# Cappucciyes/ViT-With-OpenCL

Hardware: AMD Instinct MI355X
Metric: images/sec ViT-B/16 224x224 bs512 (higher is better)
Workload: dtype f32

## Files before the change

### vit-with-opencl_amd/csrc/attention_p3.hip

```cpp
#include "kernelHandler.h"
#include "kernel_limits.h"
#include "vit_kernels.h"
#include "fp32_split.h"
#include "gemm_common.h"

namespace {

constexpr int HD = 64;
constexpr int MAX_LDS = KL_LDS_BYTES;
constexpr int MAX_ROWS = KL_ATTN_HD64_MAX_TOKENS;
static_assert(2 * 2 * 3 * MAX_ROWS * 64 <= MAX_LDS && MAX_ROWS % 16 == 0 && MAX_ROWS <= 32 * 7, "the rows of launch_k and launch_t");

typedef const __attribute__((address_space(1))) void *gptr_t;
typedef __attribute__((address_space(3))) void *lptr_t;
typedef short s16x4 __attribute__((ext_vector_type(4)));

template <int NKT, int NPL, int OUTK, bool CLSQ = false>
__global__ __launch_bounds__(64 * NKT) void attention_p3_kernel(const char *__restrict__ qkv3, char *__restrict__ out3,
                                                               unsigned char *__restrict__ aux,
                                                               int T, int E, int H, int n_items, int RB)
{
    static_assert((NPL == 3 && OUTK == 3) || (NPL == 1 && (OUTK == 4 || OUTK == 0 || OUTK == 8)), "parts / output kind");
    static_assert(!CLSQ || OUTK == 3, "the class-query variant runs on the exact planes");
    unsigned char *const out_scales = aux;
    typedef typename PartT<NPL>::type part_t;
    constexpr int NT = NPL == 3 ? 6 : 1;
    extern __shared__ __attribute__((aligned(16))) char smem[];
    const int slot = 2 * NPL * RB * 64;
    char *Kb = smem, *Vb = smem + slot;

    const int tid = threadIdx.x, lane = tid & 63;
    const int wave = __builtin_amdgcn_readfirstlane(tid >> 6);
    const int lr = lane & 31, lh = lane >> 5;
    const int E32 = E >> 5, rb16 = RB >> 4, pieces = 2 * NPL * rb16;
    const size_t prow = (size_t)(n_items / H) * T;
    const size_t orows = CLSQ ? (size_t)(n_items / H) : prow;
    const bool computes = !CLSQ || wave == 0;

    auto dma = [&](int item, int which , char *dst) {
        const int b = item / H, h = item - b * H;
        const int ks0 = which * E32 + 2 * h;
        for (int p = wave; p < pieces; p += NKT) {
            const int gp = p / rb16, rb = p - gp * rb16;
            const int r = 16 * rb + (lane >> 2);
            int c = lane & 3;
            if (which == 1)
                c ^= swz64(lane >> 4);
            const char *src = qkv3 + ((size_t)(ks0 * NPL + gp) * prow + (size_t)b * T + min(r, T - 1)) * 64 + 16 * c;
            __builtin_amdgcn_global_load_lds((gptr_t)src, (lptr_t)(dst + p * 1024), 16, 0, 0);
        }
    };

    const int q = wave * 32 + lr;
    part_t qp[HD / 16][NPL];
    auto load_q = [&](int item) {
        const int b = item / H, h = item - b * H;
        if constexpr (CLSQ) {
#pragma unroll
            for (int g = 0; g < HD / 16; ++g)
#pragma unroll
                for (int pl = 0; pl < NPL; ++pl) {
                    const f32x4 v = *reinterpret_cast<const f32x4 *>(
                        reinterpret_cast<const char *>(aux) + ((size_t)((2 * h + (g >> 1)) * NPL + pl) * orows + b) * 64 + 16 * (2 * (g & 1) + lh));
                    qp[g][pl] = __builtin_bit_cast(part_t, lr == 0 ? v : f32x4{0.0f, 0.0f, 0.0f, 0.0f});
                }
            return;
        }
        const size_t row = (size_t)b * T + min(q, T - 1);
#pragma unroll
        for (int g = 0; g < HD / 16; ++g)
#pragma unroll
            for (int pl = 0; pl < NPL; ++pl)
                qp[g][pl] = __builtin_bit_cast(part_t, *reinterpret_cast<const f32x4 *>(
                                qkv3 + ((size_t)((2 * h + (g >> 1)) * NPL + pl) * prow + row) * 64 + 16 * (2 * (g & 1) + lh)));
    };

    int kofs[2], kofs_last[2];
    {
        const int rl = min(32 * (NKT - 1) + lr, RB - 1);
#pragma unroll
        for (int gl = 0; gl < 2; ++gl) {
            kofs[gl] = lr * 64 + 16 * ((2 * gl + lh) ^ swz64(lr >> 2));
            kofs_last[gl] = rl * 64 + 16 * ((2 * gl + lh) ^ swz64(rl >> 2));
        }
    }
    const int vofs = (4 * lh + ((lane & 15) >> 2)) * 64 + ((lane & 16) + 4 * (lane & 3)) * 2;

    int item = blockIdx.x;
    if (item >= n_items)
        return;
    if (computes)
        load_q(item);
    dma(item, 1, Kb);
    __syncthreads();

    for (; item < n_items; item += gridDim.x) {
        const int b = item / H, h = item - b * H;
        const int next = item + gridDim.x;
        dma(item, 2, Vb);

        f32x16 s[NKT];
        if (computes) {
            part_t kp[3][NPL];
            auto read_k = [&](part_t (&k3)[NPL], int f) {
                const int j = f / (HD / 16), g = f % (HD / 16);
#pragma unroll
                for (int o = 0; o < NPL; ++o) {
                    const int pl = (NPL - o) % NPL;
                    const char *base = Kb + ((g >> 1) * NPL + pl) * RB * 64;
                    k3[pl] = __builtin_bit_cast(part_t, (j < NKT - 1)
                        ? *reinterpret_cast<const f32x4 *>(base + kofs[g & 1] + j * 32 * 64)
                        : *reinterpret_cast<const f32x4 *>(base + kofs_last[g & 1]));
                }
            };
            read_k(kp[0], 0);
            if (NKT * (HD / 16) > 1)
                read_k(kp[1], 1);
#pragma unroll
            for (int f = 0; f < NKT * (HD / 16); ++f) {
                const int j = f / (HD / 16), g = f % (HD / 16);
                if (g == 0) {
#pragma unroll
                    for (int r = 0; r < 16; ++r)
                        s[j][r] = 0.0f;
                }
                if (f + 2 < NKT * (HD / 16))
                    read_k(kp[(f + 2) % 3], f + 2);
#pragma unroll
                for (int t = 0; t < NT; ++t)
                    s[j] = mfma_part(kp[f % 3][term_w<NPL>(t)], qp[g][term_a<NPL>(t)], s[j]);
                if (NPL == 3) {
#pragma unroll
                    for (int r = 0; r < 3; ++r) {
                        __builtin_amdgcn_sched_group_barrier(0x100, 1, 0);
                        __builtin_amdgcn_sched_group_barrier(0x008, 2, 0);
                    }
                    __builtin_amdgcn_sched_barrier(0);
                }
            }
        }

        __syncthreads();
        if (next < n_items) {
            dma(next, 1, Kb);
            if (computes)
                load_q(next);
        }

        if (computes) {
#pragma unroll
            for (int r = 0; r < 16; ++r) {
                const int key = 32 * (NKT - 1) + (r & 3) + 8 * (r >> 2) + 4 * lh;
                s[NKT - 1][r] = key < T ? s[NKT - 1][r] : -INFINITY;
            }
            float mx = -INFINITY;
#pragma unroll
            for (int j = 0; j < NKT; ++j)
#pragma unroll
                for (int r = 0; r < 16; ++r)
                    mx = fmaxf(mx, s[j][r]);
            mx = fmaxf(mx, __shfl_xor(mx, 32));
            const float c1 = 1.44269504088896340736f / sqrtf((float)HD);
            const float c2 = -mx * c1;
            float sum = 0.0f;
#pragma unroll
            for (int j = 0; j < NKT; ++j)
#pragma unroll
                for (int r = 0; r < 16; ++r) {
                    const float e = __builtin_amdgcn_exp2f(__builtin_fmaf(s[j][r], c1, c2));
                    s[j][r] = e;
                    sum += e;
                }
            sum += __shfl_xor(sum, 32);
            const float inv_sum = 1.0f / sum;
#pragma unroll
            for (int j = 0; j < NKT; ++j)
#pragma unroll
                for (int r = 0; r < 16; ++r)
                    s[j][r] = s[j][r] * inv_sum;

            f32x16 o[2];
#pragma unroll
            for (int r = 0; r < 16; ++r) {
                o[0][r] = 0.0f;
                o[1][r] = 0.0f;
            }
            part_t vq[2][NPL], pp[NPL];
            auto read_v = [&](part_t (&v3)[NPL], int f) {
                const int j = f >> 2, t = (f >> 1) & 1, dt = f & 1;
                const int r0 = (j == NKT - 1) ? min(32 * j + 16 * t, RB - 16) : 32 * j + 16 * t;
#pragma unroll
                for (int o3 = 0; o3 < NPL; ++o3) {
                    const int pl = (NPL - o3) % NPL;
                    const char *vp = Vb + (dt * NPL + pl) * RB * 64 + r0 * 64 + vofs;
                    const s16x4 lo = __builtin_amdgcn_ds_read_tr16_b64_v4i16((__attribute__((address_space(3))) s16x4 *)(vp));
                    const s16x4 hi = __builtin_amdgcn_ds_read_tr16_b64_v4i16((__attribute__((address_space(3))) s16x4 *)(vp + 8 * 64));
                    typedef short s16x8 __attribute__((ext_vector_type(8)));
                    v3[pl] = __builtin_bit_cast(part_t, s16x8{lo[0], lo[1], lo[2], lo[3], hi[0], hi[1], hi[2], hi[3]});
                }
            };
            read_v(vq[0], 0);
#pragma unroll
            for (int f = 0; f < 4 * NKT; ++f) {
                const int j = f >> 2, t = (f >> 1) & 1, dt = f & 1;
                if (f + 1 < 4 * NKT)
                    read_v(vq[(f + 1) & 1], f + 1);
                if (dt == 0)
                    split_parts(f32x4{s[j][8 * t], s[j][8 * t + 1], s[j][8 * t + 2], s[j][8 * t + 3]},
                                f32x4{s[j][8 * t + 4], s[j][8 * t + 5], s[j][8 * t + 6], s[j][8 * t + 7]}, pp);
                if (!(j == NKT - 1 && 32 * j + 16 * t >= T)) {
#pragma unroll
                    for (int tt = 0; tt < NT; ++tt)
                        o[dt] = mfma_part(vq[f & 1][term_w<NPL>(tt)], pp[term_a<NPL>(tt)], o[dt]);
                }
            }

            if (CLSQ ? lr == 0 : q < T) {
                typedef unsigned u32x2 __attribute__((ext_vector_type(2)));
                typedef unsigned u32x4 __attribute__((ext_vector_type(4)));
                constexpr int OPL = OUTK == 3 ? 3 : 1;
#pragma unroll
                for (int dt = 0; dt < 2; ++dt) {
                    if (OUTK == 0) {
                        float *row = reinterpret_cast<float *>(out3) + ((size_t)b * T + q) * E + h * HD + 32 * dt + 4 * lh;
#pragma unroll
                        for (int g = 0; g < 4; ++g)
                            *reinterpret_cast<f32x4 *>(row + 8 * g) = f32x4{o[dt][4 * g], o[dt][4 * g + 1], o[dt][4 * g + 2], o[dt][4 * g + 3]};
                        continue;
                    }
                    if (OUTK == 8) {
                        float amax = 0.0f;
#pragma unroll
                        for (int r = 0; r < 16; ++r)
                            amax = fmaxf(amax, fabsf(o[dt][r]));
                        amax = fmaxf(amax, __shfl_xor(amax, 32));
                        unsigned sbyte;
                        float mult;
                        mx_block_scale(amax, sbyte, mult);
                        unsigned x[4];
#pragma unroll
                        for (int g = 0; g < 4; ++g)
                            x[g] = pack_fp8x4(f32x4{o[dt][4 * g], o[dt][4 * g + 1], o[dt][4 * g + 2], o[dt][4 * g + 3]} * mult);
                        const auto r02 = __builtin_amdgcn_permlane32_swap(x[0], x[2], false, false);
                        const auto r13 = __builtin_amdgcn_permlane32_swap(x[1], x[3], false, false);
                        const int col = h * HD + 32 * dt, ks = col >> 7, blk = (col >> 5) & 3;
                        const size_t row = (size_t)b * T + q;
                        *reinterpret_cast<u32x4 *>(out3 + ((size_t)ks * prow + row) * 128 + 32 * blk + 16 * lh) =
                            u32x4{r02[0], r02[1], r13[0], r13[1]};
                        if (lh == 0)
                            out_scales[mx_act_scale_index(ks, blk, row, prow)] = (unsigned char)sbyte;
                        continue;
                    }
                    u32x2 pg[4][OPL];
#pragma unroll
                    for (int g = 0; g < 4; ++g) {
                        bf16x4 part[3];
                        const f32x4 v4 = f32x4{o[dt][4 * g], o[dt][4 * g + 1], o[dt][4 * g + 2], o[dt][4 * g + 3]};
                        if (OUTK == 3) {
                            split4(v4, part[0], part[1], part[2]);
                        } else {
#pragma unroll
                            for (int e = 0; e < 4; ++e)
                                part[0][e] = (__bf16)v4[e];
                        }
#pragma unroll
                        for (int pl = 0; pl < OPL; ++pl)
                            pg[g][pl] = __builtin_bit_cast(u32x2, part[pl]);
                    }
                    char *d3 = out3 + ((size_t)(2 * h + dt) * OPL * orows + (CLSQ ? (size_t)b : (size_t)b * T + q)) * 64 + 16 * lh;
#pragma unroll
                    for (int pl = 0; pl < OPL; ++pl)
#pragma unroll
                        for (int g = 0; g < 4; g += 2) {
                            const auto r0 = __builtin_amdgcn_permlane32_swap(pg[g][pl][0], pg[g + 1][pl][0], false, false);
                            const auto r1 = __builtin_amdgcn_permlane32_swap(pg[g][pl][1], pg[g + 1][pl][1], false, false);
                            *reinterpret_cast<u32x4 *>(d3 + (size_t)pl * orows * 64 + 16 * g) = u32x4{r0[0], r1[0], r0[1], r1[1]};
                        }
                }
            }
        }

        __syncthreads();
    }
}

template <int NKT, int NPL, int OUTK, bool CLSQ>
int launch_k(hipStream_t st, const char *qkv3, char *out3, unsigned char *aux, int n_images, int T, int E, int H)
{
    const int RB = (T + 15) / 16 * 16;
    const size_t lds = (size_t)2 * 2 * NPL * RB * 64;
    VH_SET_LDS_ONCE((attention_p3_kernel<NKT, NPL, OUTK, CLSQ>), MAX_LDS);
    const int num_cus = vh_device_cus(vh_current_device());
    const int n_items = n_images * H;
    const int grid = n_items < num_cus ? n_items : num_cus;
    hipLaunchKernelGGL((attention_p3_kernel<NKT, NPL, OUTK, CLSQ>), dim3(grid), dim3(64 * NKT), lds, st, qkv3, out3, aux, T, E, H, n_items, RB);
    VH_LAUNCH_CHECK("attention_p3_kernel");
    return 0;
}


template <int NPL, int OUTK, bool CLSQ = false>
int launch_t(hipStream_t st, const char *in, char *out, unsigned char *out_scales, int n_images, int tokens, int embed_dim, int num_heads)
{
    switch ((tokens + 31) / 32) {
    case 1: return launch_k<1, NPL, OUTK, CLSQ>(st, in, out, out_scales, n_images, tokens, embed_dim, num_heads);
    case 2: return launch_k<2, NPL, OUTK, CLSQ>(st, in, out, out_scales, n_images, tokens, embed_dim, num_heads);
    case 3: return launch_k<3, NPL, OUTK, CLSQ>(st, in, out, out_scales, n_images, tokens, embed_dim, num_heads);
    case 4: return launch_k<4, NPL, OUTK, CLSQ>(st, in, out, out_scales, n_images, tokens, embed_dim, num_heads);
    case 5: return launch_k<5, NPL, OUTK, CLSQ>(st, in, out, out_scales, n_images, tokens, embed_dim, num_heads);
    case 6: return launch_k<6, NPL, OUTK, CLSQ>(st, in, out, out_scales, n_images, tokens, embed_dim, num_heads);
    default: return launch_k<7, NPL, OUTK, CLSQ>(st, in, out, out_scales, n_images, tokens, embed_dim, num_heads);
    }
}

int check_args(const char *who, const void *in, const void *out, int n_images, int tokens, int embed_dim, int num_heads)
{
    if (!in || !out)
        return vh_fail(1, "%s: null pointer argument", who);
    if (n_images <= 0 || tokens <= 0 || num_heads <= 0 || embed_dim != num_heads * HD || tokens > MAX_ROWS)
        return vh_fail(1, "%s: needs head_dim 64 and 1 <= tokens <= %d (n=%d tokens=%d embed=%d heads=%d)", who,
                       MAX_ROWS, n_images, tokens, embed_dim, num_heads);
    if ((((uintptr_t)in | (uintptr_t)out) & 15) != 0)
        return vh_fail(1, "%s: pointers must be 16-byte aligned", who);
    return 0;
}

}

extern "C" int vh_launch_attention_planes(vh_stream_t s, const void *qkv_planes, void *out_planes, int n_images,
                                          int tokens, int embed_dim, int num_heads)
{
    if (int rc = check_args("vh_launch_attention_planes", qkv_planes, out_planes, n_images, tokens, embed_dim, num_heads))
        return rc;
    return launch_t<3, 3>((hipStream_t)s, static_cast<const char *>(qkv_planes), static_cast<char *>(out_planes), nullptr,
                          n_images, tokens, embed_dim, num_heads);
}

extern "C" int vh_launch_attention_planes_cls(vh_stream_t s, const void *qkv_planes, const void *q_cls_planes, void *out_cls_planes,
                                              int n_images, int tokens, int embed_dim, int num_heads)
{
    if (int rc = check_args("vh_launch_attention_planes_cls", qkv_planes, out_cls_planes, n_images, tokens, embed_dim, num_heads))
        return rc;
    if (!q_cls_planes || ((uintptr_t)q_cls_planes & 15) != 0)
        return vh_fail(1, "vh_launch_attention_planes_cls: q_cls_planes must be a 16-byte aligned pointer");
    return launch_t<3, 3, true>((hipStream_t)s, static_cast<const char *>(qkv_planes), static_cast<char *>(out_cls_planes),
                                static_cast<unsigned char *>(const_cast<void *>(q_cls_planes)), n_images, tokens, embed_dim, num_heads);
}

extern "C" int vh_launch_attention_planes_f16(vh_stream_t s, const void *qkv_planes_f16, void *output, int output_planes,
                                              int n_images, int tokens, int embed_dim, int num_heads)
{
    if (int rc = check_args("vh_launch_attention_planes_f16", qkv_planes_f16, output, n_images, tokens, embed_dim, num_heads))
        return rc;
    const char *in = static_cast<const char *>(qkv_planes_f16);
    char *out = static_cast<char *>(output);
    return output_planes ? launch_t<1, 4>((hipStream_t)s, in, out, nullptr, n_images, tokens, embed_dim, num_heads)
                         : launch_t<1, 0>((hipStream_t)s, in, out, nullptr, n_images, tokens, embed_dim, num_heads);
}

extern "C" int vh_launch_attention_planes_f16_mx(vh_stream_t s, const void *qkv_planes_f16, void *out_values, void *out_scales,
                                                 int n_images, int tokens, int embed_dim, int num_heads)
{
    if (int rc = check_args("vh_launch_attention_planes_f16_mx", qkv_planes_f16, out_values, n_images, tokens, embed_dim, num_heads))
        return rc;
    if (!out_scales || embed_dim % 128 != 0)
        return vh_fail(1, "vh_launch_attention_planes_f16_mx: needs out_scales and embed_dim %% 128 == 0");
    return launch_t<1, 8>((hipStream_t)s, static_cast<const char *>(qkv_planes_f16), static_cast<char *>(out_values),
                          static_cast<unsigned char *>(out_scales), n_images, tokens, embed_dim, num_heads);
}
```

### vit-with-opencl_amd/csrc/kernel_limits.h

```cpp
#ifndef VIT_KERNEL_LIMITS_H
#define VIT_KERNEL_LIMITS_H

#include "kernelHandler.h"

#include <stddef.h>

#ifdef __cplusplus
#define KL_FN static constexpr
#else
#define KL_FN static inline
#endif

enum { KL_LDS_BYTES = 160 * 1024 };

enum {
    KL_ATTN_HD64_MAX_TOKENS = 208,
    KL_ATTN_HD80_MAX_TOKENS = 272,
    KL_ATTN_STREAMING_MAX_TOKENS = 512
};
KL_FN int kl_attn_long_head_dim_ok(int head_dim) { return head_dim == 64 || head_dim == 80; }

enum { KL_LN_PLANES_ROWS = 16, KL_LN_PLANES_MAX_EMBED = 2048 };
KL_FN int kl_layer_norm_planes_max_embed(int parts)
{
    if (parts != 1 && parts != 3)
        return 0;
    const int by_lds = KL_LDS_BYTES / (parts * KL_LN_PLANES_ROWS * 64) * 32;
    return by_lds < KL_LN_PLANES_MAX_EMBED ? by_lds : KL_LN_PLANES_MAX_EMBED;
}

enum { KL_FOLD_GROUP = 128, KL_FOLD_MAX_GROUPS = 16 };

enum {
    KL_PATCH_PLANES_K_STEP = 128,
    KL_PATCH_ROWS_K_STEP = 32
};
KL_FN int kl_patch_planes_k(int in_chans, int patch_size)
{
    const int K = in_chans * patch_size * patch_size, step = KL_PATCH_PLANES_K_STEP;
    return (K + step - 1) / step * step;
}
KL_FN int kl_patch_direct(int in_chans, int img_w, int patch_size)
{
    return patch_size % 4 == 0 && (in_chans * patch_size * patch_size) % KL_PATCH_ROWS_K_STEP == 0 && img_w % 4 == 0;
}
KL_FN size_t kl_patch_rows_workspace(int n_images, int in_chans, int img_h, int img_w, int patch_size, int embed_dim)
{
    if (n_images <= 0 || in_chans <= 0 || img_h <= 0 || img_w <= 0 || patch_size <= 0 || embed_dim <= 0 ||
        img_h % patch_size != 0 || img_w % patch_size != 0 || kl_patch_direct(in_chans, img_w, patch_size))
        return 0;
    const size_t np = (size_t)(img_h / patch_size) * (size_t)(img_w / patch_size), K = (size_t)in_chans * patch_size * patch_size;
    const size_t Kp = (K + KL_PATCH_ROWS_K_STEP - 1) / KL_PATCH_ROWS_K_STEP * KL_PATCH_ROWS_K_STEP;
    return ((size_t)n_images * np + (size_t)embed_dim) * Kp * sizeof(float);
}

KL_FN size_t kl_mx_act_scale_bytes(int rows, int cols)
{
    return rows > 0 && cols > 0 ? (size_t)((cols / 128 + 3) / 4) * 16 * (size_t)rows : 0;
}

enum { KL_CLS_ATTN_MAX_HEAD_DIM = 128 };
KL_FN int kl_cls_attention_head_dim_ok(int head_dim)
{
    return head_dim > 0 && head_dim % 16 == 0 && head_dim <= KL_CLS_ATTN_MAX_HEAD_DIM;
}

enum { KL_ROLLOUT_QUERY_ROWS = 16, KL_ROLLOUT_KEY_CHUNK = 64 };
KL_FN size_t kl_rollout_workspace(int n_images, int tokens)
{
    return n_images > 0 && tokens > 0 ? (size_t)n_images * (size_t)tokens * (size_t)tokens * sizeof(float) : 0;
}
KL_FN int kl_rollout_score_stride(int tokens)
{
    return (tokens + KL_ROLLOUT_KEY_CHUNK - 1) / KL_ROLLOUT_KEY_CHUNK * KL_ROLLOUT_KEY_CHUNK + 20;
}
KL_FN size_t kl_rollout_lds_bytes(int tokens, int head_dim)
{
    return ((size_t)KL_ROLLOUT_QUERY_ROWS * kl_rollout_score_stride(tokens) +
            (size_t)(KL_ROLLOUT_QUERY_ROWS + KL_ROLLOUT_KEY_CHUNK) * (head_dim + 4)) * sizeof(float);
}
KL_FN int kl_rollout_max_tokens(int head_dim)
{
    int T = 0;
    while (kl_rollout_lds_bytes(T + KL_ROLLOUT_KEY_CHUNK, head_dim) <= (size_t)KL_LDS_BYTES)
        T += KL_ROLLOUT_KEY_CHUNK;
    return T;
}

enum { KL_GALLERY_ROW_TILE = 128, KL_GALLERY_MAX_EMBED = 2048 };
KL_FN size_t kl_gallery_workspace(int n_queries, long n_rows, int k, int splits)
{
    if (n_queries < 1 || n_rows < 1 || k < 1 || splits < 0)
        return 0;
    if (splits == 0) {
        const long tiles = (n_rows + KL_GALLERY_ROW_TILE - 1) / KL_GALLERY_ROW_TILE;
        splits = tiles < VH_GALLERY_MAX_SPLITS ? (int)tiles : VH_GALLERY_MAX_SPLITS;
    }
    return (size_t)n_queries * (size_t)splits * (size_t)k * sizeof(unsigned long long);
}

enum { KL_READOUT_ROWS = 32 };
KL_FN size_t kl_feature_readout_scratch(int n_images, int tokens, int embed_dim)
{
    if (n_images <= 0 || tokens < 2 || embed_dim <= 0)
        return 0;
    return (size_t)n_images * ((tokens - 1 + KL_READOUT_ROWS - 1) / KL_READOUT_ROWS) * embed_dim * sizeof(float);
}

enum { KL_DENSE_MAX_EMBED = 2048 };

KL_FN size_t kl_round16(size_t v) { return (v + 15) & ~(size_t)15; }
KL_FN size_t kl_dense_stitch_scratch(int n_windows, int frame_h, int frame_w, long n_ids)
{
    if (n_windows < 1 || frame_h < 1 || frame_w < 1 || frame_h > VH_STITCH_MAX_SIDE || frame_w > VH_STITCH_MAX_SIDE || n_ids < 0 ||
        n_ids > 2147483647L)
        return 0;
    const size_t blocks = (size_t)((frame_h + VH_STITCH_BLOCK - 1) / VH_STITCH_BLOCK) * (size_t)((frame_w + VH_STITCH_BLOCK - 1) / VH_STITCH_BLOCK);
    return kl_round16((size_t)n_windows * 16) + kl_round16((blocks + 1) * sizeof(int)) + kl_round16((size_t)n_ids * sizeof(int)) + 16;
}

#endif
```

Baseline: 6441.

## Stream class-query attention through a per-wave triple-buffered LDS ring

Adds a dedicated class-token attention kernel in which each wave owns one (image, head) item. K and V tiles are streamed through a three-slot LDS ring with two tiles in flight, using vmcnt waits, and the next item's tiles are prefetched. This replaces the old path, where a whole workgroup loaded all K/V but only wave 0 computed. It also rebalances DMA piece assignment across waves for the 7-wave full-attention kernel, so that some waves issue no loads. In exchange it brings more hand-written waitcnt and inline-asm transposed LDS reads, which carry correctness risk.

Measured after the change: 6480 (median of 6 runs). About the same (+0.6%).

```diff
diff --git a/vit-with-opencl_amd/csrc/attention_p3.hip b/vit-with-opencl_amd/csrc/attention_p3.hip
--- a/vit-with-opencl_amd/csrc/attention_p3.hip
+++ b/vit-with-opencl_amd/csrc/attention_p3.hip
@@ -14,6 +14,22 @@
 typedef const __attribute__((address_space(1))) void *gptr_t;
 typedef __attribute__((address_space(3))) void *lptr_t;
 typedef short s16x4 __attribute__((ext_vector_type(4)));
+
+#ifndef ATTN_DMA_ROLES
+#define ATTN_DMA_ROLES 1
+#endif
+#ifndef ATTN_CLSQ_STREAM
+#define ATTN_CLSQ_STREAM 1
+#endif
+struct DmaShare { int first, count; };
+template <int NKT, bool BY_WAITERS> struct DmaRoles {
+    static constexpr int SLOTS = NKT;
+    static __device__ __forceinline__ DmaShare of(int wave) { return DmaShare{wave, 1}; }
+};
+template <> struct DmaRoles<7, true> {
+    static constexpr int SLOTS = 5;
+    static __device__ __forceinline__ DmaShare of(int wave) { return DmaShare{wave < 4 ? wave : 0, wave < 3 ? 1 : wave == 3 ? 2 : 0}; }
+};
 
 template <int NKT, int NPL, int OUTK, bool CLSQ = false>
 __global__ __launch_bounds__(64 * NKT) void attention_p3_kernel(const char *__restrict__ qkv3, char *__restrict__ out3,
@@ -36,11 +52,14 @@
     const size_t prow = (size_t)(n_items / H) * T;
     const size_t orows = CLSQ ? (size_t)(n_items / H) : prow;
     const bool computes = !CLSQ || wave == 0;
+    typedef DmaRoles<NKT, ATTN_DMA_ROLES && NPL == 3 && !CLSQ> ROLES;
+    const DmaShare roles = ROLES::of(wave);
 
     auto dma = [&](int item, int which , char *dst) {
         const int b = item / H, h = item - b * H;
         const int ks0 = which * E32 + 2 * h;
-        for (int p = wave; p < pieces; p += NKT) {
+        for (int sl = 0; sl < roles.count; ++sl)
+        for (int p = roles.first + sl; p < pieces; p += ROLES::SLOTS) {
             const int gp = p / rb16, rb = p - gp * rb16;
             const int r = 16 * rb + (lane >> 2);
             int c = lane & 3;
@@ -298,6 +317,267 @@
     return 0;
 }
 
+constexpr int CQ_WAVES = KL_ATTN_CLSQ_WAVES, CQ_RING = KL_ATTN_CLSQ_RING, CQ_TILE = KL_ATTN_CLSQ_TILE_BYTES;
+constexpr int CQ_PIECES = CQ_TILE / 1024;
+static_assert(CQ_TILE == 2 * 3 * 32 * HD && CQ_RING == 3 && 2 * CQ_PIECES < 64, "ring of three tiles, two in flight on a 6-bit vmcnt");
+static_assert(CQ_WAVES * (CQ_RING * CQ_TILE + 1024) == KL_ATTN_CLSQ_LDS_BYTES && KL_ATTN_CLSQ_LDS_BYTES <= MAX_LDS, "the LDS of launch_cls_k");
+
+template <int N> __device__ __forceinline__ void wait_vm() { asm volatile("s_waitcnt vmcnt(%0)" ::"n"(N) : "memory"); }
+
+__device__ __forceinline__ void read_v_tr3(const char *vp, bf16x8 (&v3)[3])
+{
+    const unsigned addr = (unsigned)(uintptr_t)(__attribute__((address_space(3))) const char *)vp;
+    s16x4 lo[3], hi[3];
+    asm volatile("ds_read_b64_tr_b16 %0, %6\n\t"
+                 "ds_read_b64_tr_b16 %1, %6 offset:512\n\t"
+                 "ds_read_b64_tr_b16 %2, %6 offset:2048\n\t"
+                 "ds_read_b64_tr_b16 %3, %6 offset:2560\n\t"
+                 "ds_read_b64_tr_b16 %4, %6 offset:4096\n\t"
+                 "ds_read_b64_tr_b16 %5, %6 offset:4608\n\t"
+                 "s_waitcnt lgkmcnt(0)"
+                 : "=&v"(lo[0]), "=&v"(hi[0]), "=&v"(lo[1]), "=&v"(hi[1]), "=&v"(lo[2]), "=&v"(hi[2])
+                 : "v"(addr)
+                 : "memory");
+    typedef short s16x8 __attribute__((ext_vector_type(8)));
+#pragma unroll
+    for (int pl = 0; pl < 3; ++pl)
+        v3[pl] = __builtin_bit_cast(bf16x8, s16x8{lo[pl][0], lo[pl][1], lo[pl][2], lo[pl][3], hi[pl][0], hi[pl][1], hi[pl][2], hi[pl][3]});
+}
+
+template <int NKT>
+__global__ __launch_bounds__(64 * CQ_WAVES) void attention_p3_cls_kernel(const char *__restrict__ qkv3, char *__restrict__ out3,
+                                                                        const char *__restrict__ qcls, int T, int E, int H, int n_items)
+{
+    constexpr int NPL = 3, NT = 6, NTILES = 2 * NKT;
+    typedef bf16x8 part_t;
+    extern __shared__ __attribute__((aligned(16))) char smem[];
+
+    const int lane = threadIdx.x & 63;
+    const int wave = __builtin_amdgcn_readfirstlane(threadIdx.x >> 6);
+    const int lr = lane & 31, lh = lane >> 5;
+    const int E32 = E >> 5;
+    const size_t prow = (size_t)(n_items / H) * T;
+    const size_t orows = (size_t)(n_items / H);
+    const int stride = gridDim.x * CQ_WAVES;
+    int item = blockIdx.x * CQ_WAVES + wave;
+    if (item >= n_items)
+        return;
+
+    int slot[CQ_RING];
+#pragma unroll
+    for (int r = 0; r < CQ_RING; ++r)
+        slot[r] = (wave * CQ_RING + r) * CQ_TILE;
+
+    auto issue = [&](int it, int tl, int dst) {
+        const int b = it / H, h = it - b * H;
+        const int which = tl < NKT ? 1 : 2, j = tl < NKT ? tl : tl - NKT;
+        const int ks0 = which * E32 + 2 * h;
+        int c = lane & 3;
+        if (which == 1)
+            c ^= swz64(lane >> 4);
+#pragma unroll
+        for (int pc = 0; pc < CQ_PIECES; ++pc) {
+            const int gp = pc >> 1, rb = pc & 1;
+            const int r = 32 * j + 16 * rb + (lane >> 2);
+            const char *src = qkv3 + ((size_t)(ks0 * NPL + gp) * prow + (size_t)b * T + min(r, T - 1)) * 64 + 16 * c;
+            __builtin_amdgcn_global_load_lds((gptr_t)src, (lptr_t)(smem + dst + pc * 1024), 16, 0, 0);
+        }
+    };
+
+    const int qslot = CQ_WAVES * CQ_RING * CQ_TILE + wave * 1024;
+    part_t qp[HD / 16][NPL];
+    auto issue_q = [&](int it) {
+        const int b = it / H, h = it - b * H;
+        const int ch = min(lane, 23), g = ch / 6, pl = (ch >> 1) % 3, half = ch & 1;
+        const char *src = qcls + ((size_t)((2 * h + (g >> 1)) * NPL + pl) * orows + b) * 64 + 16 * (2 * (g & 1) + half);
+        __builtin_amdgcn_global_load_lds((gptr_t)src, (lptr_t)(smem + qslot), 16, 0, 0);
+    };
+    auto read_q = [&]() {
+#pragma unroll
+        for (int g = 0; g < HD / 16; ++g)
+#pragma unroll
+            for (int pl = 0; pl < NPL; ++pl) {
+                const f32x4 v = *reinterpret_cast<const f32x4 *>(smem + qslot + 16 * ((3 * g + pl) * 2 + lh));
+                qp[g][pl] = __builtin_bit_cast(part_t, lr == 0 ? v : f32x4{0.0f, 0.0f, 0.0f, 0.0f});
+            }
+    };
+
+    int kofs[2];
+#pragma unroll
+    for (int gl = 0; gl < 2; ++gl)
+        kofs[gl] = lr * 64 + 16 * ((2 * gl + lh) ^ swz64(lr >> 2));
+    const int vofs = (4 * lh + ((lane & 15) >> 2)) * 64 + ((lane & 16) + 4 * (lane & 3)) * 2;
+
+    auto advance = [&](int i , int next) {
+        asm volatile("s_waitcnt lgkmcnt(0)" ::: "memory");
+        if (i + 2 < NTILES) {
+            issue(item, i + 2, slot[2]);
+            wait_vm<2 * CQ_PIECES>();
+        } else if (next < n_items) {
+            issue(next, i + 2 - NTILES, slot[2]);
+            wait_vm<2 * CQ_PIECES>();
+        } else if (i + 1 < NTILES) {
+            wait_vm<CQ_PIECES>();
+        } else {
+            wait_vm<0>();
+        }
+    };
+    auto rotate = [&]() {
+        const int s0 = slot[0];
+        slot[0] = slot[1];
+        slot[1] = slot[2];
+        slot[2] = s0;
+    };
+
+    issue_q(item);
+    issue(item, 0, slot[0]);
+    if (NTILES > 1)
+        issue(item, 1, slot[1]);
+
+    for (; item < n_items; item += stride) {
+        const int b = item / H, h = item - b * H;
+        const int next = item + stride;
+
+        f32x16 s[NKT];
+#pragma unroll
+        for (int j = 0; j < NKT; ++j) {
+            advance(j, next);
+            if (j == 0)
+                read_q();
+            const char *tile = smem + slot[0];
+            part_t kp[HD / 16][NPL];
+#pragma unroll
+            for (int g = 0; g < HD / 16; ++g)
+#pragma unroll
+                for (int pl = 0; pl < NPL; ++pl)
+                    kp[g][pl] = __builtin_bit_cast(part_t, *reinterpret_cast<const f32x4 *>(tile + ((g >> 1) * NPL + pl) * 2048 + kofs[g & 1]));
+#pragma unroll
+            for (int r = 0; r < 16; ++r)
+                s[j][r] = 0.0f;
+#pragma unroll
+            for (int g = 0; g < HD / 16; ++g)
+#pragma unroll
+                for (int t = 0; t < NT; ++t)
+                    s[j] = mfma_part(kp[g][term_w<NPL>(t)], qp[g][term_a<NPL>(t)], s[j]);
+            rotate();
+        }
+        if (next < n_items)
+            issue_q(next);
+
+#pragma unroll
+        for (int r = 0; r < 16; ++r) {
+            const int key = 32 * (NKT - 1) + (r & 3) + 8 * (r >> 2) + 4 * lh;
+            s[NKT - 1][r] = key < T ? s[NKT - 1][r] : -INFINITY;
+        }
+        float mx = -INFINITY;
+#pragma unroll
+        for (int j = 0; j < NKT; ++j)
+#pragma unroll
+            for (int r = 0; r < 16; ++r)
+                mx = fmaxf(mx, s[j][r]);
+        mx = fmaxf(mx, __shfl_xor(mx, 32));
+        const float c1 = 1.44269504088896340736f / sqrtf((float)HD);
+        const float c2 = -mx * c1;
+        float sum = 0.0f;
+#pragma unroll
+        for (int j = 0; j < NKT; ++j)
+#pragma unroll
+            for (int r = 0; r < 16; ++r) {
+                const float e = __builtin_amdgcn_exp2f(__builtin_fmaf(s[j][r], c1, c2));
+                s[j][r] = e;
+                sum += e;
+            }
+        sum += __shfl_xor(sum, 32);
+        const float inv_sum = 1.0f / sum;
+#pragma unroll
+        for (int j = 0; j < NKT; ++j)
+#pragma unroll
+            for (int r = 0; r < 16; ++r)
+                s[j][r] = s[j][r] * inv_sum;
+
+        f32x16 o[2];
+#pragma unroll
+        for (int r = 0; r < 16; ++r) {
+            o[0][r] = 0.0f;
+            o[1][r] = 0.0f;
+        }
+#pragma unroll
+        for (int j = 0; j < NKT; ++j) {
+            advance(NKT + j, next);
+            const char *tile = smem + slot[0];
+#pragma unroll
+            for (int t = 0; t < 2; ++t) {
+                if (j == NKT - 1 && 32 * j + 16 * t >= T)
+                    continue;
+                part_t pp[NPL];
+                split_parts(f32x4{s[j][8 * t], s[j][8 * t + 1], s[j][8 * t + 2], s[j][8 * t + 3]},
+                            f32x4{s[j][8 * t + 4], s[j][8 * t + 5], s[j][8 * t + 6], s[j][8 * t + 7]}, pp);
+#pragma unroll
+                for (int dt = 0; dt < 2; ++dt) {
+                    part_t vq[NPL];
+                    read_v_tr3(tile + dt * NPL * 2048 + 16 * t * 64 + vofs, vq);
+#pragma unroll
+                    for (int tt = 0; tt < NT; ++tt)
+                        o[dt] = mfma_part(vq[term_w<NPL>(tt)], pp[term_a<NPL>(tt)], o[dt]);
+                }
+            }
+            rotate();
+        }
+
+        if (lr == 0) {
+            typedef unsigned u32x2 __attribute__((ext_vector_type(2)));
+            typedef unsigned u32x4 __attribute__((ext_vector_type(4)));
+#pragma unroll
+            for (int dt = 0; dt < 2; ++dt) {
+                u32x2 pg[4][NPL];
+#pragma unroll
+                for (int g = 0; g < 4; ++g) {
+                    bf16x4 part[3];
+                    split4(f32x4{o[dt][4 * g], o[dt][4 * g + 1], o[dt][4 * g + 2], o[dt][4 * g + 3]}, part[0], part[1], part[2]);
+#pragma unroll
+                    for (int pl = 0; pl < NPL; ++pl)
+                        pg[g][pl] = __builtin_bit_cast(u32x2, part[pl]);
+                }
+                char *d3 = out3 + ((size_t)(2 * h + dt) * NPL * orows + (size_t)b) * 64 + 16 * lh;
+#pragma unroll
+                for (int pl = 0; pl < NPL; ++pl)
+#pragma unroll
+                    for (int g = 0; g < 4; g += 2) {
+                        const auto r0 = __builtin_amdgcn_permlane32_swap(pg[g][pl][0], pg[g + 1][pl][0], false, false);
+                        const auto r1 = __builtin_amdgcn_permlane32_swap(pg[g][pl][1], pg[g + 1][pl][1], false, false);
+                        *reinterpret_cast<u32x4 *>(d3 + (size_t)pl * orows * 64 + 16 * g) = u32x4{r0[0], r1[0], r0[1], r1[1]};
+                    }
+            }
+        }
+    }
+}
+
+
+template <int NKT>
+int launch_cls_k(hipStream_t st, const char *qkv3, char *out3, const char *qcls, int n_images, int T, int E, int H)
+{
+    VH_SET_LDS_ONCE((attention_p3_cls_kernel<NKT>), KL_ATTN_CLSQ_LDS_BYTES);
+    const int num_cus = vh_device_cus(vh_current_device());
+    const int n_items = n_images * H;
+    const int wgs = (n_items + CQ_WAVES - 1) / CQ_WAVES;
+    const int grid = wgs < num_cus ? wgs : num_cus;
+    hipLaunchKernelGGL((attention_p3_cls_kernel<NKT>), dim3(grid), dim3(64 * CQ_WAVES), KL_ATTN_CLSQ_LDS_BYTES, st, qkv3, out3, qcls, T, E, H, n_items);
+    VH_LAUNCH_CHECK("attention_p3_cls_kernel");
+    return 0;
+}
+
+int launch_cls(hipStream_t st, const char *in, char *out, const char *qcls, int n_images, int tokens, int embed_dim, int num_heads)
+{
+    switch ((tokens + 31) / 32) {
+    case 1: return launch_cls_k<1>(st, in, out, qcls, n_images, tokens, embed_dim, num_heads);
+    case 2: return launch_cls_k<2>(st, in, out, qcls, n_images, tokens, embed_dim, num_heads);
+    case 3: return launch_cls_k<3>(st, in, out, qcls, n_images, tokens, embed_dim, num_heads);
+    case 4: return launch_cls_k<4>(st, in, out, qcls, n_images, tokens, embed_dim, num_heads);
+    case 5: return launch_cls_k<5>(st, in, out, qcls, n_images, tokens, embed_dim, num_heads);
+    case 6: return launch_cls_k<6>(st, in, out, qcls, n_images, tokens, embed_dim, num_heads);
+    default: return launch_cls_k<7>(st, in, out, qcls, n_images, tokens, embed_dim, num_heads);
+    }
+}
 
 template <int NPL, int OUTK, bool CLSQ = false>
 int launch_t(hipStream_t st, const char *in, char *out, unsigned char *out_scales, int n_images, int tokens, int embed_dim, int num_heads)
@@ -343,8 +623,13 @@
         return rc;
     if (!q_cls_planes || ((uintptr_t)q_cls_planes & 15) != 0)
         return vh_fail(1, "vh_launch_attention_planes_cls: q_cls_planes must be a 16-byte aligned pointer");
+#if ATTN_CLSQ_STREAM
+    return launch_cls((hipStream_t)s, static_cast<const char *>(qkv_planes), static_cast<char *>(out_cls_planes),
+                      static_cast<const char *>(q_cls_planes), n_images, tokens, embed_dim, num_heads);
+#else
     return launch_t<3, 3, true>((hipStream_t)s, static_cast<const char *>(qkv_planes), static_cast<char *>(out_cls_planes),
                                 static_cast<unsigned char *>(const_cast<void *>(q_cls_planes)), n_images, tokens, embed_dim, num_heads);
+#endif
 }
 
 extern "C" int vh_launch_attention_planes_f16(vh_stream_t s, const void *qkv_planes_f16, void *output, int output_planes,
diff --git a/vit-with-opencl_amd/csrc/kernel_limits.h b/vit-with-opencl_amd/csrc/kernel_limits.h
--- a/vit-with-opencl_amd/csrc/kernel_limits.h
+++ b/vit-with-opencl_amd/csrc/kernel_limits.h
@@ -17,6 +17,12 @@
     KL_ATTN_HD64_MAX_TOKENS = 208,
     KL_ATTN_HD80_MAX_TOKENS = 272,
     KL_ATTN_STREAMING_MAX_TOKENS = 512
+};
+enum {
+    KL_ATTN_CLSQ_WAVES = 4,
+    KL_ATTN_CLSQ_RING = 3,
+    KL_ATTN_CLSQ_TILE_BYTES = 2 * 3 * 32 * 64,
+    KL_ATTN_CLSQ_LDS_BYTES = KL_ATTN_CLSQ_WAVES * (KL_ATTN_CLSQ_RING * KL_ATTN_CLSQ_TILE_BYTES + 1024)
 };
 KL_FN int kl_attn_long_head_dim_ok(int head_dim) { return head_dim == 64 || head_dim == 80; }
 
```
